# Yotsuei/ClearConverse

Measured on AMD Instinct MI355X. Metric: xRT (audio-sec/wall-sec) end-to-end, 30 s 16 kHz clips, higher is better.
Workload: dtype bf16

## Files before the change

clearconverse_amd/_lib.py:

```python
from __future__ import annotations

import ctypes as C
import os
from pathlib import Path
from typing import Optional

_PKG = Path(__file__).resolve().parent
LIB_PATH = _PKG / "libccx.so"


class CcxError(RuntimeError):
    pass


class WhisperDims(C.Structure):
    _fields_ = [(n, C.c_int) for n in (
        "n_mels", "n_audio_ctx", "n_audio_state", "n_audio_head", "n_audio_layer",
        "n_vocab", "n_text_ctx", "n_text_state", "n_text_head", "n_text_layer")]


class SepformerDims(C.Structure):
    _fields_ = [(n, C.c_int) for n in (
        "n_filters", "kernel", "stride", "d_model", "n_head", "d_ffn", "n_layers", "n_blocks", "segment", "n_spk")]

# ... 59 lines not shown
        + [(n, C.c_int64) for n in ("h_elems", "xin_elems", "y_elems", "qkv_elems", "att_elems", "feats_elems", "fc_elems")]
        + [("rows", C.c_int), ("seq_start", C.POINTER(C.c_int)), ("seq_len", C.POINTER(C.c_int)), ("n_seq", C.c_int),
           ("n_tok", C.c_int), ("d_ffn", C.c_int)]
        + [(n, C.c_void_p) for n in ("ln_g", "ln_b", "gln_g", "gln_b", "wqkv", "bqkv", "wo", "bo", "w1", "b1", "w2", "b2", "wdec")]
        + [(n, C.c_int64) for n in ("ln_elems", "gln_elems", "wqkv_elems", "bqkv_elems", "wo_elems", "bo_elems", "w1_elems",
                                    "b1_elems", "w2_elems", "b2_elems", "wdec_elems")]
        + [("utt_tok0", C.POINTER(C.c_int)), ("utt_L", C.POINTER(C.c_int)), ("utt_T", C.POINTER(C.c_int)), ("n_utt", C.c_int),
           ("segment", C.c_int), ("out", C.c_void_p), ("out_stride", C.c_int64), ("out_elems", C.c_int64)])


SEP_ATTN_BLOCK, SEP_ATTENTION, SEP_FFN, SEP_FINAL_NORM, SEP_DECODER = range(5)


class AlignDesc(C.Structure):
    _fields_ = [
        ("q", C.c_void_p), ("k", C.c_void_p), ("q_elems", C.c_int64), ("k_elems", C.c_int64),
        ("n_seq", C.c_int), ("H", C.c_int), ("Spad", C.c_int),
        ("heads", C.POINTER(C.c_int)), ("n_heads", C.c_int), ("head0", C.c_int), ("t", C.c_int),
        ("Hsel", C.c_int), ("T", C.c_int), ("Mmax", C.c_int),
        ("n_keys", C.POINTER(C.c_int)), ("n_rows", C.POINTER(C.c_int)), ("r0", C.c_int),
        ("P", C.c_void_p), ("A", C.c_void_p), ("P_elems", C.c_int64), ("A_elems", C.c_int64),
        ("text_idx", C.c_void_p), ("time_idx", C.c_void_p), ("path_len", C.c_void_p), ("jump_frame", C.c_void_p),
        ("text_idx_elems", C.c_int64), ("time_idx_elems", C.c_int64), ("path_len_elems", C.c_int64), ("jump_frame_elems", C.c_int64)]


ALIGN_SCORES, ALIGN_MATRIX, ALIGN_DTW = range(3)


_vp, _i, _i64, _f = C.c_void_p, C.c_int, C.c_int64, C.c_float
_ip = C.POINTER(C.c_int)
_i32p = C.POINTER(C.c_int32)
_i64p = C.POINTER(C.c_int64)
_fp = C.POINTER(C.c_float)

PROTOTYPES = {
    "ccx_version": (C.c_char_p, []),
    "ccx_ctx_create": (_i, [_i, C.POINTER(_vp)]),
    "ccx_ctx_destroy": (None, [_vp]),
    "ccx_last_error": (C.c_char_p, [_vp]),
    "ccx_prof_enable": (_i, [_vp, _i]),
    "ccx_prof_count": (_i, [_vp]),
    "ccx_prof_get": (_i, [_vp, _i, C.c_char_p, _i, C.POINTER(C.c_double), C.POINTER(C.c_double), _fp]),
    "ccx_gemm_bf16": (_i, [_vp, _i, _vp, _i64, _vp, _i64, _vp, _vp, _i64, _vp, _i64, _i, _i, _i, _vp]),
    "ccx_gemm_bf16_desc": (_i, [_vp, _i, C.POINTER(GemmDesc), _vp]),
    "ccx_layernorm": (_i, [_vp, _vp, _vp, _vp, _vp, _vp, _i, _i, _f, _vp]),
    "ccx_gather_rows": (_i, [_vp, _vp, _vp, _i, _i, _vp, _i64, _vp]),
    "ccx_peak_normalize": (_i, [_vp, _vp, _vp, _i64, _vp, _i, _f, _vp]),
    "ccx_row_variance": (_i, [_vp, _vp, _i64, _vp, _i, _vp, _vp]),
    "ccx_cross_attention_xa": (_i, [_vp, _vp, _vp, _vp, _vp, _vp, _vp, _i, _i, _i, _i, _i, _vp, _vp]),
    "ccx_cosine_rows": (_i, [_vp, _vp, _vp, _i, _i, _i, _vp, _vp]),
    "ccx_speaker_profiles": (_i, [_vp, _vp, _vp, _vp, _i, _i, _i, _i, _vp, _vp]),
    "ccx_resample_sinc": (_i, [_vp, _vp, _i64, _vp, _i, _i, _i, _i, _vp, _vp, _i64, _vp, _i, _vp]),
    "ccx_enc_attention": (_i, [_vp, _vp, _vp, _vp, _vp, _i, _i, _i, _i, _vp]),
    "ccx_whisper_create": (_i, [_vp, C.POINTER(WhisperDims), _i, C.POINTER(_vp)]),
    "ccx_whisper_destroy": (None, [_vp]),
    "ccx_whisper_set_tensor": (_i, [_vp, C.c_char_p, _vp, _i, _i, _i64p]),
    "ccx_whisper_set_max_audio": (_i, [_vp, C.c_double]),
    "ccx_whisper_share_encoder_scratch": (_i, [_vp, _vp]),
    "ccx_whisper_finalize": (_i, [_vp]),
    "ccx_whisper_set_rules": (_i, [_vp, C.POINTER(DecodeRules)]),
    "ccx_whisper_logmel": (_i, [_vp, _vp, _i64, _ip, _ip, _i, _vp, _vp]),
    "ccx_whisper_set_mel": (_i, [_vp, _vp, _i, _vp]),
    "ccx_whisper_encode": (_i, [_vp, _i, _vp, _vp]),
    "ccx_whisper_decoder_logits": (_i, [_vp, _i32p, _i, _i, _vp, _vp]),
    "ccx_whisper_decode_greedy": (_i, [_vp, _i32p, _i32p, _i, _i, _i, _i32p, _i32p, _fp, _fp, _vp]),
    "ccx_dec_attention_desc": (_i, [_vp, _i, C.POINTER(DecAttnDesc), _vp]),
    "ccx_dec_select_step": (_i, [_vp, C.POINTER(DecSelectDesc), _vp]),
    "ccx_align_op": (_i, [_vp, _i, C.POINTER(AlignDesc), _vp]),
    "ccx_whisper_align": (_i, [_vp, _i32p, _i32p, _i, _i, _i32p, _i32p, _i, _i, _vp, _vp, _i32p, _vp]),
    "ccx_whisper_last_cross_path": (_i, [_vp]),
    "ccx_whisper_prepare_lanes": (_i, [_vp, _vp]),
    "ccx_whisper_trace_lanes": (_i, [_vp, C.c_char_p, _i]),
    "ccx_whisper_decode": (_i, [_vp, _i32p, _i32p, _i, _i, _i, _f, C.c_uint64, _i32p, _i32p, _fp, _fp, _vp]),
    "ccx_sepformer_create": (_i, [_vp, C.POINTER(SepformerDims), _i, _i, C.POINTER(_vp)]),
    "ccx_sepformer_destroy": (None, [_vp]),
    "ccx_sepformer_set_tensor": (_i, [_vp, C.c_char_p, _vp, _i64]),
    "ccx_sepformer_finalize": (_i, [_vp]),
    "ccx_sepformer_separate": (_i, [_vp, _vp, _i64, _ip, _i, _vp, _vp]),
    "ccx_sep_op": (_i, [_vp, _i, C.POINTER(SepDesc), _vp]),
    "ccx_speaker_create": (_i, [_vp, _i, _i, _i, _i, _i64, C.POINTER(_vp)]),
    "ccx_speaker_destroy": (None, [_vp]),
    "ccx_speaker_set_tensor": (_i, [_vp, C.c_char_p, _vp, _i64]),
    "ccx_speaker_finalize": (_i, [_vp]),
    "ccx_speaker_embed": (_i, [_vp, _vp, _i64p, _ip, _i, _vp, _i64p, _ip, _vp, _vp]),
    "ccx_speaker_segment": (_i, [_vp, _vp, _i64p, _ip, _i, _vp, _i64, _ip, _vp]),
    "ccx_resnet_create": (_i, [_vp, _i, _i64, _i, C.POINTER(_vp)]),
    "ccx_resnet_destroy": (None, [_vp]),
    "ccx_resnet_set_tensor": (_i, [_vp, C.c_char_p, _vp, _i64]),
    "ccx_resnet_finalize": (_i, [_vp]),
    "ccx_resnet_embed": (_i, [_vp, _vp, _i64, _i, _i, _vp, _i, _ip, _i, _vp, _vp]),
    "ccx_specgate_create": (_i, [_vp, _i64, _i, _i, C.POINTER(_vp)]),
    "ccx_specgate_destroy": (None, [_vp]),
    "ccx_specgate_reduce": (_i, [_vp, _vp, _i64, _ip, _i, _f, _vp, _vp]),
    "ccx_specgate_reduce_long": (_i, [_vp, _vp, _i64, _f, _vp, _vp]),
    "ccx_specgate_set_clip_noise": (_i, [_vp, _i]),
}

_lib: Optional[C.CDLL] = None


def load() -> C.CDLL:
    global _lib
    if _lib is not None:
        return _lib
    if not LIB_PATH.exists():
        raise CcxError(f"{LIB_PATH} is missing: run `python -m clearconverse_amd.build` "
# ... 71 lines not shown
```

clearconverse_amd/csrc/api.hip:

```cpp
#include <stdarg.h>
#include "../../include/ccx.h"
#include "attention.h"
#include "ccx_common.h"
#include "elementwise.h"
#include "gemm_bf16.h"

static thread_local std::string g_create_error;

int ccx_fail(ccx_ctx* ctx, int code, const char* fmt, ...) {
  char buf[1024];
  va_list ap;
  va_start(ap, fmt);
  vsnprintf(buf, sizeof(buf), fmt, ap);
  va_end(ap);
  if (ctx) {
    std::lock_guard<std::mutex> lk(ctx->mu);
    ctx->last_error = buf;
  } else g_create_error = buf;
  return code;
}

extern "C" {

const char* ccx_version(void) { return "ccx 0.1 (gfx950)"; }
// ... 112 lines not shown
      if (rrow > max_rrow) max_rrow = rrow;
    }
    const long o_need = max_orow < 0 ? 0 : max_orow * p.ldo + Nw;
    CCX_REQUIRE(ctx, o_need <= d->out_elems, "ccx_gemm_bf16_desc: out is written up to element %ld, out_elems=%ld", o_need, (long)d->out_elems);
    const bool res_f32 = epi == EPI_F32_RESID || epi == EPI_F32_GELU_POS || epi == EPI_BF16_LRELU_AFFINE;
    if (res_f32 && p.resid) {
      const long r_need = max_rrow * p.ldr + Nw;
      CCX_REQUIRE(ctx, r_need <= d->resid_elems, "ccx_gemm_bf16_desc: resid is read up to element %ld, resid_elems=%ld", r_need, (long)d->resid_elems);
    }
    if (epi == EPI_BF16_ADD_RELU && p.resid_bf16) {
      const long r_need = max_rrow * p.ldrb + Nw;
      CCX_REQUIRE(ctx, r_need <= d->resid_bf16_elems, "ccx_gemm_bf16_desc: resid_bf16 is read up to element %ld, resid_bf16_elems=%ld", r_need,
                  (long)d->resid_bf16_elems);
    }
  }
  return ccx_launch_gemm(ctx, epi, p, (hipStream_t)stream);
}

int ccx_layernorm(ccx_ctx* ctx, const float* x, const float* gamma, const float* beta, void* out_bf16, float* out_f32,
                  int M, int D, float eps, void* stream) {
  if (!ctx) return CCX_ERR_ARG;
  return ccx_launch_layernorm(ctx, x, D, gamma, beta, (bf16_t*)out_bf16, out_f32, D, M, D, eps, (hipStream_t)stream);
}

int ccx_peak_normalize(ccx_ctx* ctx, const float* x, float* y, int64_t stride, const int* n_samples_dev, int B, float eps, void* stream) {
  if (!ctx) return CCX_ERR_ARG;
  return ccx_launch_peak_normalize(ctx, x, y, (long)stride, n_samples_dev, B, eps, (hipStream_t)stream);
}

int ccx_row_variance(ccx_ctx* ctx, const float* x, int64_t stride, const int* n_samples_dev, int B, float* out, void* stream) {
  if (!ctx) return CCX_ERR_ARG;
  return ccx_launch_row_variance(ctx, x, (long)stride, n_samples_dev, B, out, (hipStream_t)stream);
}

int ccx_cosine_rows(ccx_ctx* ctx, const float* a, const float* b, int R, int D, int b_rows, float* out, void* stream) {
  if (!ctx) return CCX_ERR_ARG;
  return ccx_launch_cosine_rows(ctx, a, b, R, D, b_rows, out, (hipStream_t)stream);
}

int ccx_speaker_profiles(ccx_ctx* ctx, const float* emb, const float* w, const int* spk_dev, int C, int T, int D, int S, float* out, void* stream) {
  if (!ctx) return CCX_ERR_ARG;
  return ccx_launch_speaker_profiles(ctx, emb, w, spk_dev, C, T, D, S, out, (hipStream_t)stream);
}

int ccx_gather_rows(ccx_ctx* ctx, const int64_t* src_ptrs_dev, const int* lens_dev, int n_rows, int max_len, float* dst_dev,
                    int64_t stride, void* stream) {
  if (!ctx) return CCX_ERR_ARG;
  return ccx_launch_gather_rows(ctx, (const long*)src_ptrs_dev, lens_dev, n_rows, max_len, dst_dev, (long)stride, (hipStream_t)stream);
}

int ccx_enc_attention(ccx_ctx* ctx, const void* q, const void* k, const void* vt, void* o, int B, int H, int S, int Spad,
                      void* stream) {
  if (!ctx) return CCX_ERR_ARG;
  return ccx_launch_enc_attention(ctx, (const bf16_t*)q, (const bf16_t*)k, (const bf16_t*)vt, (bf16_t*)o, B, H, S, Spad,
                                  (hipStream_t)stream);
}

}
```

clearconverse_amd/csrc/attention.h:

```cpp
#pragma once
#include "ccx_common.h"

int ccx_launch_enc_attention(ccx_ctx* ctx, const bf16_t* Q, const bf16_t* K, const bf16_t* Vt, bf16_t* O,
                             int B, int n_head, int S, int Spad, hipStream_t stream);
```

clearconverse_amd/csrc/attention.hip:

```cpp
#include <type_traits>
#include "attention.h"

typedef const __attribute__((address_space(1))) void* gptr_t;
typedef __attribute__((address_space(3))) void* lptr_t;

#define ATT_STAGE 16384

__global__ __launch_bounds__(256, 2) void enc_attention_kernel(
    const bf16_t* __restrict__ Q, const bf16_t* __restrict__ Kc, const bf16_t* __restrict__ Vt,
    bf16_t* __restrict__ O, int S, int Spad, int n_head, float scale_log2e, int n_qt) {
  __shared__ __attribute__((aligned(16))) char smem[2 * ATT_STAGE];
  const int tid = threadIdx.x, lane = tid & 63, wave = tid >> 6;
  const int nwg = gridDim.x, orig = blockIdx.x;
  const int xcd = orig & 7, qq = nwg >> 3, rr = nwg & 7;
  const int wg = (xcd < rr ? xcd * (qq + 1) : rr * (qq + 1) + (xcd - rr) * qq) + (orig >> 3);
  const int bh = wg / n_qt;
  const int q0 = (wg - bh * n_qt) * 128 + wave * 32;
  const int l31 = lane & 31, hh = lane >> 5;

  const bf16_t* Qb = Q + (long)bh * Spad * 64;
  const bf16_t* Kb = Kc + (long)bh * Spad * 64;
  const bf16_t* Vb = Vt + (long)bh * 64 * Spad;

  bf16x8 qf[4];
  {
    int qr = q0 + l31; qr = qr < Spad ? qr : Spad - 1;
#pragma unroll
    for (int ds = 0; ds < 4; ds++) qf[ds] = *(const bf16x8*)(Qb + (long)qr * 64 + 16 * ds + 8 * hh);
  }

  const bf16_t* srcK[2];
  const bf16_t* srcV[2];
#pragma unroll
  for (int i = 0; i < 2; i++) {
    const int inst = wave * 2 + i;
    const int r = inst * 8 + (lane >> 3);
    const int c = (lane & 7) ^ ((r >> 1) & 7);
    srcK[i] = Kb + (long)r * 64 + c * 8;
    srcV[i] = Vb + (long)r * Spad + c * 8;
  }
  auto stage = [&](int t, int buf) {
    char* sK = smem + buf * ATT_STAGE;
    char* sV = sK + 8192;
#pragma unroll
    for (int i = 0; i < 2; i++) {
      const int inst = wave * 2 + i;
      __builtin_amdgcn_global_load_lds((gptr_t)(srcK[i] + (long)t * 64 * 64), (lptr_t)(sK + inst * 1024), 16, 0, 0);
      __builtin_amdgcn_global_load_lds((gptr_t)(srcV[i] + (long)t * 64), (lptr_t)(sV + inst * 1024), 16, 0, 0);
    }
  };

  const int prow = (l31 & ~0xC) | (((l31 >> 2) & 1) << 3) | (((l31 >> 3) & 1) << 2);
  int offK[4], offV[4];
#pragma unroll
  for (int s = 0; s < 4; s++) {
    offK[s] = prow * 128 + (((2 * s + hh) ^ ((prow >> 1) & 7)) << 4);
    offV[s] = l31 * 128 + (((2 * s + hh) ^ ((l31 >> 1) & 7)) << 4);
  }

  f32x16 oT[2];
#pragma unroll
  for (int i = 0; i < 16; i++) { oT[0][i] = 0.f; oT[1][i] = 0.f; }
  float m_run = -1e30f, l_run = 0.f;

  const int nT = (S + 63) >> 6;
  const f32x16 zero16 = {0.f, 0.f, 0.f, 0.f, 0.f, 0.f, 0.f, 0.f, 0.f, 0.f, 0.f, 0.f, 0.f, 0.f, 0.f, 0.f};
  auto tile = [&](int t, auto tail_tag) {
    constexpr bool TAIL = decltype(tail_tag)::value;
    const int buf = t & 1;
    if (t + 1 < nT) stage(t + 1, buf ^ 1);
    const char* sK = smem + buf * ATT_STAGE;
    const char* sV = sK + 8192;

    f32x16 sT[2];
#pragma unroll
    for (int kt = 0; kt < 2; kt++) {
#pragma unroll
      for (int ds = 0; ds < 4; ds++) {
        const bf16x8 kf = *(const bf16x8*)(sK + kt * 32 * 128 + offK[ds]);
        sT[kt] = __builtin_amdgcn_mfma_f32_32x32x16_bf16(kf, qf[ds], ds == 0 ? zero16 : sT[kt], 0, 0, 0);
      }
    }
    float mx = -1e30f;
#pragma unroll
    for (int kt = 0; kt < 2; kt++)
#pragma unroll
      for (int r = 0; r < 16; r++) {
        if (TAIL) {
          const int key = t * 64 + kt * 32 + 16 * (r >> 3) + 8 * hh + (r & 7);
          if (key >= S) sT[kt][r] = -INFINITY;
        }
        mx = fmaxf(mx, sT[kt][r]);
      }
    mx = fmaxf(mx, __shfl_xor(mx, 32, 64));
    const float m_new = fmaxf(m_run, mx * scale_log2e);
    const float alpha = __builtin_amdgcn_exp2f(m_run - m_new);
    m_run = m_new;
    float psum = 0.f;
#pragma unroll
    for (int kt = 0; kt < 2; kt++)
#pragma unroll
      for (int r = 0; r < 16; r++) {
        const float pv = __builtin_amdgcn_exp2f(fmaf(sT[kt][r], scale_log2e, -m_new));
        sT[kt][r] = pv;
        psum += pv;
      }
    l_run = l_run * alpha + psum;
    if (__builtin_amdgcn_ballot_w64(alpha != 1.f) != 0) {
#pragma unroll
      for (int i = 0; i < 16; i++) { oT[0][i] *= alpha; oT[1][i] *= alpha; }
    }

    bf16x8 pf[4];
#pragma unroll
    for (int kt = 0; kt < 2; kt++)
#pragma unroll
      for (int s = 0; s < 2; s++) {
        union { bf16x8 v; uint32_t u[4]; } cv;
#pragma unroll
        for (int j = 0; j < 4; j++) cv.u[j] = pack_bf16x2(sT[kt][8 * s + 2 * j], sT[kt][8 * s + 2 * j + 1]);
        pf[2 * kt + s] = cv.v;
      }
#pragma unroll
    for (int dt = 0; dt < 2; dt++)
#pragma unroll
      for (int ks = 0; ks < 4; ks++) {
        const bf16x8 vf = *(const bf16x8*)(sV + dt * 32 * 128 + offV[ks]);
        oT[dt] = __builtin_amdgcn_mfma_f32_32x32x16_bf16(vf, pf[ks], oT[dt], 0, 0, 0);
      }
    __syncthreads();
  };
  stage(0, 0);
  __syncthreads();
  for (int t = 0; t < nT - 1; t++) tile(t, std::false_type{});
  if ((S & 63) != 0) tile(nT - 1, std::true_type{});
  else tile(nT - 1, std::false_type{});

  const float l_tot = l_run + __shfl_xor(l_run, 32, 64);
  const float inv = 1.0f / l_tot;
  const int q = q0 + l31;
  if (q < S) {
    const int b = bh / n_head, h = bh - b * n_head;
    bf16_t* dst = O + ((long)(b * S + q) * n_head + h) * 64;
#pragma unroll
    for (int dt = 0; dt < 2; dt++)
#pragma unroll
      for (int g = 0; g < 4; g++) {
        uint2 v;
        v.x = pack_bf16x2(oT[dt][4 * g + 0] * inv, oT[dt][4 * g + 1] * inv);
        v.y = pack_bf16x2(oT[dt][4 * g + 2] * inv, oT[dt][4 * g + 3] * inv);
        *(uint2*)(dst + dt * 32 + 8 * g + 4 * hh) = v;
      }
  }
}

int ccx_launch_enc_attention(ccx_ctx* ctx, const bf16_t* Q, const bf16_t* K, const bf16_t* Vt, bf16_t* O,
                             int B, int n_head, int S, int Spad, hipStream_t stream) {
  CCX_REQUIRE(ctx, B > 0 && n_head > 0 && S > 0, "enc_attention: empty problem");
  CCX_REQUIRE(ctx, Spad % 64 == 0 && Spad >= S, "enc_attention: Spad=%d must be a multiple of 64 and >= S=%d", Spad, S);
  const float scale_log2e = 0.125f * 1.4426950408889634f;
  const int n_qt = ccx_cdiv(S, 128);
  dim3 grid(n_qt * B * n_head);
  {
    const double bh = (double)B * n_head;
    ccx_prof_scope ps(ctx, stream, "enc_attention_kernel", 4.0 * bh * S * (double)S * 64, 2.0 * bh * S * 64 * 4);
    hipLaunchKernelGGL(enc_attention_kernel, grid, dim3(256), 0, stream, Q, K, Vt, O, S, Spad, n_head, scale_log2e, n_qt);
  }
  CCX_CHECK_LAUNCH(ctx);
  return CCX_OK;
}
```

clearconverse_amd/csrc/whisper.hip:

```cpp
#include <array>
#include <atomic>
#include <map>
#include <chrono>
#include <math.h>
#include "../../include/ccx.h"
#include "align.h"
#include "attention.h"
#include "ccx_common.h"
#include "cross_x.h"
#include "decoder.h"
#include "elementwise.h"
#include "gemm_bf16.h"
#include "logmel.h"
#include "model_store.h"

namespace {

struct EncLayer {
  float *ln1_g, *ln1_b, *ln2_g, *ln2_b;
  bf16_t *Wqkv, *Wo, *W1, *W2;
  float *bqkv, *bo, *b1, *b2;
};
struct DecLayer {
  float *ln1_g, *ln1_b, *lnc_g, *lnc_b, *ln2_g, *ln2_b;
// ... 255 lines not shown

int ccx_whisper_trace_lanes(ccx_whisper* w, const char* path, int level) {
  CCX_REQUIRE(w->ctx, w->finalized, "whisper: trace_lanes before finalize");
  w->stamps_on = path != nullptr && path[0] != 0;
  w->stamp_path = w->stamps_on ? path : "";
  w->stamp_level = level >= 2 ? 2 : 1;
  CCX_HIP(w->ctx, hipMemset(w->stamp_count, 0, ccx_whisper::kMaxLanes * 4));
  for (auto& g : w->graphs) hipGraphExecDestroy(g.second);
  w->graphs.clear();
  return CCX_OK;
}

int ccx_whisper_finalize(ccx_whisper* w) {
  if (!w) return CCX_ERR_ARG;
  CCX_REQUIRE(w->ctx, !w->finalized, "whisper: finalize called twice");
  CCX_HIP(w->ctx, hipSetDevice(w->ctx->device));
  const ccx_whisper_dims& d = w->d;
  const int D = d.n_audio_state, F = 4 * D, B = w->max_batch, S = d.n_audio_ctx, H = d.n_audio_head;
  CCX_TRY(w->store.open_arena((size_t)64 << 20));
  CCX_TRY(build_logmel_tables(w));

  {
    CCX_NEED(w->store, c1w, "encoder.conv1.weight", D, d.n_mels, 3);
    CCX_NEED(w->store, c1b, "encoder.conv1.bias", D);
    CCX_NEED(w->store, c2w, "encoder.conv2.weight", D, D, 3);
    CCX_NEED(w->store, c2b, "encoder.conv2.bias", D);
    CCX_NEED(w->store, pe, "encoder.positional_embedding", S, D);
    CCX_NEED(w->store, lg, "encoder.ln_post.weight", D);
    CCX_NEED(w->store, lb, "encoder.ln_post.bias", D);
    std::vector<float> g1 = conv_to_gemm(*c1w, 256), g2 = conv_to_gemm(*c2w, 3 * D);
    CCX_TRY(w->store.upload_bf16(&w->Wc1, g1));
    CCX_TRY(w->store.upload_bf16(&w->Wc2, g2));
    CCX_TRY(w->store.upload(&w->bc1, c1b->data.data(), D));
    CCX_TRY(w->store.upload(&w->bc2, c2b->data.data(), D));
    CCX_TRY(w->store.upload(&w->enc_pos, pe->data.data(), (size_t)S * D));
    CCX_TRY(w->store.upload(&w->lnp_g, lg->data.data(), D));
    CCX_TRY(w->store.upload(&w->lnp_b, lb->data.data(), D));
  }
  w->enc.resize(d.n_audio_layer);
  const std::vector<float> zerosD(D, 0.f);
  for (int l = 0; l < d.n_audio_layer; l++) {
    const std::string p = "encoder.blocks." + std::to_string(l) + ".";
    EncLayer& L = w->enc[l];
    CCX_NEED(w->store, qw, p + "attn.query.weight", D, D); CCX_NEED(w->store, qbias, p + "attn.query.bias", D);
    CCX_NEED(w->store, kw, p + "attn.key.weight", D, D);
    CCX_NEED(w->store, vw, p + "attn.value.weight", D, D); CCX_NEED(w->store, vbias, p + "attn.value.bias", D);
    CCX_NEED(w->store, ow, p + "attn.out.weight", D, D); CCX_NEED(w->store, obias, p + "attn.out.bias", D);
    CCX_NEED(w->store, l1g, p + "attn_ln.weight", D); CCX_NEED(w->store, l1b, p + "attn_ln.bias", D);
    CCX_NEED(w->store, m0w, p + "mlp.0.weight", F, D); CCX_NEED(w->store, m0b, p + "mlp.0.bias", F);
    CCX_NEED(w->store, m2w, p + "mlp.2.weight", D, F); CCX_NEED(w->store, m2b, p + "mlp.2.bias", D);
    CCX_NEED(w->store, l2g, p + "mlp_ln.weight", D); CCX_NEED(w->store, l2b, p + "mlp_ln.bias", D);
    std::vector<float> wqkv = cat_rows({&qw->data, &kw->data, &vw->data});
    std::vector<float> bqkv = cat_rows({&qbias->data, &zerosD, &vbias->data});
    CCX_TRY(w->store.upload_bf16(&L.Wqkv, wqkv)); CCX_TRY(w->store.upload(&L.bqkv, bqkv));
    CCX_TRY(w->store.upload_bf16(&L.Wo, ow->data)); CCX_TRY(w->store.upload(&L.bo, obias->data.data(), D));
    CCX_TRY(w->store.upload_bf16(&L.W1, m0w->data)); CCX_TRY(w->store.upload(&L.b1, m0b->data.data(), F));
    CCX_TRY(w->store.upload_bf16(&L.W2, m2w->data)); CCX_TRY(w->store.upload(&L.b2, m2b->data.data(), D));
    CCX_TRY(w->store.upload(&L.ln1_g, l1g->data.data(), D)); CCX_TRY(w->store.upload(&L.ln1_b, l1b->data.data(), D));
    CCX_TRY(w->store.upload(&L.ln2_g, l2g->data.data(), D)); CCX_TRY(w->store.upload(&L.ln2_b, l2b->data.data(), D));
  }

  {
    CCX_NEED(w->store, te, "decoder.token_embedding.weight", d.n_vocab, D);
    CCX_NEED(w->store, pe, "decoder.positional_embedding", d.n_text_ctx, D);
    CCX_NEED(w->store, lg, "decoder.ln.weight", D);
    CCX_NEED(w->store, lb, "decoder.ln.bias", D);
    CCX_TRY(w->store.upload(&w->tok_emb_f32, te->data));
    CCX_TRY(w->store.upload_bf16(&w->tok_emb_rm, te->data.data(), (size_t)d.n_vocab * D));
    CCX_TRY(w->store.upload(&w->dec_pos, pe->data));
    CCX_TRY(w->store.upload(&w->lnd_g, lg->data.data(), D));
    CCX_TRY(w->store.upload(&w->lnd_b, lb->data.data(), D));
  }
  w->dec.resize(d.n_text_layer);
  const int Tc = d.n_text_ctx;
  {
    const char* e = getenv("CCX_CROSS_X");
    w->xs_on = (!e || atoi(e) != 0) && d.n_text_state == D && d.n_text_head == H && ccx_xs_supported(D, H);
    w->kv_cap = w->xs_on ? (B < ccx_whisper::kKvSeqs ? B : ccx_whisper::kKvSeqs) : B;
  }
  for (int l = 0; l < d.n_text_layer; l++) {
    const std::string p = "decoder.blocks." + std::to_string(l) + ".";
    DecLayer& L = w->dec[l];
    CCX_NEED(w->store, qw, p + "attn.query.weight", D, D); CCX_NEED(w->store, qbias, p + "attn.query.bias", D);
    CCX_NEED(w->store, kw, p + "attn.key.weight", D, D);
    CCX_NEED(w->store, vw, p + "attn.value.weight", D, D); CCX_NEED(w->store, vbias, p + "attn.value.bias", D);
    CCX_NEED(w->store, ow, p + "attn.out.weight", D, D); CCX_NEED(w->store, obias, p + "attn.out.bias", D);
    CCX_NEED(w->store, l1g, p + "attn_ln.weight", D); CCX_NEED(w->store, l1b, p + "attn_ln.bias", D);
    CCX_NEED(w->store, cqw, p + "cross_attn.query.weight", D, D); CCX_NEED(w->store, cqb, p + "cross_attn.query.bias", D);
    CCX_NEED(w->store, ckw, p + "cross_attn.key.weight", D, D);
    CCX_NEED(w->store, cvw, p + "cross_attn.value.weight", D, D); CCX_NEED(w->store, cvb, p + "cross_attn.value.bias", D);
    CCX_NEED(w->store, cow, p + "cross_attn.out.weight", D, D); CCX_NEED(w->store, cob, p + "cross_attn.out.bias", D);
    CCX_NEED(w->store, lcg, p + "cross_attn_ln.weight", D); CCX_NEED(w->store, lcb, p + "cross_attn_ln.bias", D);
    CCX_NEED(w->store, m0w, p + "mlp.0.weight", F, D); CCX_NEED(w->store, m0b, p + "mlp.0.bias", F);
    CCX_NEED(w->store, m2w, p + "mlp.2.weight", D, F); CCX_NEED(w->store, m2b, p + "mlp.2.bias", D);
    CCX_NEED(w->store, l2g, p + "mlp_ln.weight", D); CCX_NEED(w->store, l2b, p + "mlp_ln.bias", D);
    std::vector<float> wqkv = cat_rows({&qw->data, &kw->data, &vw->data});
    std::vector<float> bqkv = cat_rows({&qbias->data, &zerosD, &vbias->data});
    std::vector<float> wckv = cat_rows({&ckw->data, &cvw->data});
    std::vector<float> bckv = cat_rows({&zerosD, &cvb->data});
    CCX_TRY(up_bf16_packed(w, &L.Wqkv, wqkv.data(), 3 * D, D, 16)); CCX_TRY(w->store.upload(&L.bqkv, bqkv));
    CCX_TRY(up_bf16_packed(w, &L.Wo, ow->data.data(), D, D, 16)); CCX_TRY(w->store.upload(&L.bo, obias->data.data(), D));
    { double sb = 0.0; for (int k = 0; k < D; k++) sb += obias->data[k]; L.bo_mean = (float)(sb / D); }
    CCX_TRY(up_bf16_packed(w, &L.Wcq, cqw->data.data(), D, D, 16)); CCX_TRY(w->store.upload(&L.bcq, cqb->data.data(), D));
    CCX_TRY(w->store.upload_bf16(&L.Wckv, wckv)); CCX_TRY(w->store.upload(&L.bckv, bckv));
    CCX_TRY(up_bf16_packed(w, &L.Wco, cow->data.data(), D, D, 16)); CCX_TRY(w->store.upload(&L.bco, cob->data.data(), D));
    CCX_TRY(up_bf16_packed(w, &L.W1, m0w->data.data(), F, D, 16)); CCX_TRY(w->store.upload(&L.b1, m0b->data.data(), F));
// ... 195 lines not shown
  CCX_REQUIRE(w->ctx, n <= w->kv_cap, "whisper: cross K/V caches hold %d sequences, %d asked for", w->kv_cap, n);
  GemmParams p;
  for (int l = 0; l < d.n_text_layer; l++) {
    const DecLayer& L = w->dec[l];
    memset(&p, 0, sizeof(p));
    p.A = w->xa; p.lda = D; p.W = L.Wckv; p.ldw = D; p.M = n * S; p.N = 2 * D; p.K = D; p.bias = L.bckv;
    p.hk = L.crossK; p.hv = L.crossV; p.d_model = D; p.n_head = H; p.S = S; p.Spad = w->Spad; p.v_transposed = 0;
    p.first_block = 1;
    CCX_TRY(ccx_launch_gemm(w->ctx, EPI_HEADS, p, stream));
  }
  w->kv_ready = n;
  return CCX_OK;
}
static void read_chain_switches(ccx_whisper* w) {
  { const char* e = getenv("CCX_FUSE_CROSS_Q"); w->fuse_cross_q = e ? (atoi(e) != 0) : 1; }
  { const char* e = getenv("CCX_DEC_LNFREE"); w->lnfree = !(e && strcmp(e, "0") == 0); }
  { const char* e = getenv("CCX_XS_FUSE_Q"); w->xs_fuse_q = !e || atoi(e) != 0; }
}
static int select_cross_path(ccx_whisper* w, int B, hipStream_t stream) {
  const char* e = getenv("CCX_CROSS_X_MIN_ROWS");
  const int min_rows = e ? atoi(e) : ccx_whisper::kKvSeqs + 1;
  w->xs_active = w->xs_on && (B >= min_rows || B > w->kv_cap);
  if (w->xs_on && !w->xs_active && w->kv_ready < B) CCX_TRY(project_cross_kv(w, B, stream));
  return CCX_OK;
}

int ccx_whisper_encode(ccx_whisper* w, int B, float* xa_out, void* stream_) {
  if (!w) return CCX_ERR_ARG;
  hipStream_t stream = (hipStream_t)stream_;
  ccx_ctx* ctx = w->ctx;
  CCX_REQUIRE(ctx, w->finalized, "whisper: not finalized");
  CCX_REQUIRE(ctx, B >= 1 && B <= w->max_batch, "whisper_encode: B=%d out of range (max %d)", B, w->max_batch);
  const ccx_whisper_dims& d = w->d;
  const int D = d.n_audio_state, F = 4 * D, S = d.n_audio_ctx, H = d.n_audio_head;
  GemmParams p;
  memset(&p, 0, sizeof(p));
  p.A = w->im2col; p.lda = 256; p.W = w->Wc1; p.ldw = 256; p.M = B * 3000; p.N = D; p.K = 256;
  p.bias = w->bc1; p.out = w->h1; p.ldo = D; p.rpb_in = 3000; p.rpb_out = 3002; p.roff = 1; p.rpb_valid = 3000;
  CCX_TRY(ccx_launch_gemm(ctx, EPI_BF16_GELU, p, stream));
  memset(&p, 0, sizeof(p));
  p.A = w->h1; p.lda = 2 * D; p.W = w->Wc2; p.ldw = 3 * D; p.M = B * 1501; p.N = D; p.K = 3 * D;
  p.bias = w->bc2; p.out = w->x; p.ldo = D; p.resid = w->enc_pos; p.ldr = D; p.resid_mod = S;
  p.rpb_in = 1501; p.rpb_out = S; p.roff = 0; p.rpb_valid = S;
  CCX_TRY(ccx_launch_gemm(ctx, EPI_F32_GELU_POS, p, stream));

  const int M = B * S;
  for (int l = 0; l < d.n_audio_layer; l++) {
    const EncLayer& L = w->enc[l];
    CCX_TRY(ccx_launch_layernorm(ctx, w->x, D, L.ln1_g, L.ln1_b, w->xn, nullptr, D, M, D, 1e-5f, stream));
    memset(&p, 0, sizeof(p));
    p.A = w->xn; p.lda = D; p.W = L.Wqkv; p.ldw = D; p.M = M; p.N = 3 * D; p.K = D; p.bias = L.bqkv;
    p.hq = w->qb; p.hk = w->kb; p.hv = w->vtb; p.d_model = D; p.n_head = H; p.S = S; p.Spad = w->Spad; p.v_transposed = 1;
    CCX_TRY(ccx_launch_gemm(ctx, EPI_HEADS, p, stream));
    CCX_TRY(ccx_launch_enc_attention(ctx, w->qb, w->kb, w->vtb, w->attn, B, H, S, w->Spad, stream));
    memset(&p, 0, sizeof(p));
    p.A = w->attn; p.lda = D; p.W = L.Wo; p.ldw = D; p.M = M; p.N = D; p.K = D; p.bias = L.bo;
    p.out = w->x; p.ldo = D; p.resid = w->x; p.ldr = D;
    CCX_TRY(ccx_launch_gemm(ctx, EPI_F32_RESID, p, stream));
    CCX_TRY(ccx_launch_layernorm(ctx, w->x, D, L.ln2_g, L.ln2_b, w->xn, nullptr, D, M, D, 1e-5f, stream));
    memset(&p, 0, sizeof(p));
    p.A = w->xn; p.lda = D; p.W = L.W1; p.ldw = D; p.M = M; p.N = F; p.K = D; p.bias = L.b1; p.out = w->ffn; p.ldo = F;
    CCX_TRY(ccx_launch_gemm(ctx, EPI_BF16_GELU, p, stream));
    memset(&p, 0, sizeof(p));
    p.A = w->ffn; p.lda = F; p.W = L.W2; p.ldw = F; p.M = M; p.N = D; p.K = F; p.bias = L.b2;
    p.out = w->x; p.ldo = D; p.resid = w->x; p.ldr = D;
    CCX_TRY(ccx_launch_gemm(ctx, EPI_F32_RESID, p, stream));
  }
  CCX_TRY(ccx_launch_layernorm(ctx, w->x, D, w->lnp_g, w->lnp_b, w->xa, xa_out, D, M, D, 1e-5f, stream));
  CCX_TRY(scratch_release(w, stream));
  w->kv_ready = 0;
  if (!w->xs_on) CCX_TRY(project_cross_kv(w, B, stream));
  return CCX_OK;
}

}

namespace {

__global__ void dec_stamp_kernel(unsigned long long* trace, int* count, int cap, int tag) {
  const int i = atomicAdd(count, 1);
  if (i < cap) trace[i] = (__builtin_amdgcn_s_memrealtime() << 8) | (unsigned long long)(tag & 255);
}

__global__ void lane_probe_spin(int* sink, long cycles) {
  const long t0 = __builtin_amdgcn_s_memtime();
  while (__builtin_amdgcn_s_memtime() - t0 < cycles) {}
  if (sink && threadIdx.x == 0) atomicAdd(sink, 1);
}

double lane_probe_time(ccx_whisper* w, hipStream_t a, hipStream_t b) {
  hipStreamSynchronize(a);
  if (b) hipStreamSynchronize(b);
  const auto t0 = std::chrono::steady_clock::now();
  for (int k = 0; k < 4; k++) {
    hipLaunchKernelGGL(lane_probe_spin, dim3(1), dim3(64), 0, a, w->probe_sink, 120000L);
    if (b) hipLaunchKernelGGL(lane_probe_spin, dim3(1), dim3(64), 0, b, w->probe_sink + 1, 120000L);
  }
  hipStreamSynchronize(a);
  if (b) hipStreamSynchronize(b);
  return std::chrono::duration<double, std::micro>(std::chrono::steady_clock::now() - t0).count();
}

const std::vector<hipStream_t>& lane_streams_for(ccx_whisper* w, hipStream_t s0, int want) {
  auto it = w->lane_sets.find(s0);
  if (it != w->lane_sets.end()) return it->second;
  (void)want;
  std::vector<hipStream_t>& set = w->lane_sets[s0];
// ... 617 lines not shown
```

include/ccx.h:

```cpp
#ifndef CCX_H
#define CCX_H
#include <stdint.h>
#ifdef __cplusplus
extern "C" {
#endif

#define CCX_DTYPE_F32 0
#define CCX_DTYPE_BF16 1
#define CCX_DTYPE_F16 2

typedef struct ccx_ctx ccx_ctx;
typedef struct ccx_whisper ccx_whisper;

const char* ccx_version(void);
int ccx_ctx_create(int device, ccx_ctx** out);
void ccx_ctx_destroy(ccx_ctx* ctx);
const char* ccx_last_error(const ccx_ctx* ctx);

int ccx_prof_enable(ccx_ctx* ctx, int on);
int ccx_prof_count(ccx_ctx* ctx);
int ccx_prof_get(ccx_ctx* ctx, int i, char* name_out, int name_cap, double* flops, double* bytes, float* ms);


int ccx_gemm_bf16(ccx_ctx* ctx, int epi, const void* A_dev, int64_t lda, const void* W_dev, int64_t ldw,
                  const float* bias_dev, void* out_dev, int64_t ldo, const float* resid_dev, int64_t ldr,
                  int M, int N, int K, void* stream);

typedef struct ccx_gemm_desc {
  const void* A; const void* W;
  int64_t lda, ldw;
  int M, N, K;
  int ntaps; int64_t a_tap_stride;
  const void* bias;
  const void* out;
  int64_t ldo;
  const void* resid;
  int64_t ldr;
  int resid_mod;
  const void* scale; const void* shift;
  float slope;
  int rpb_in, rpb_out, roff, rpb_valid;
  int img_rows_in, img_rows_valid, img_rows_out;
  const void* resid_bf16; int64_t ldrb;
  const void* hq; const void* hk; const void* hv;
  int d_model, n_head;
  int S, Spad;
  int v_transposed;
  int first_block;
  int64_t a_elems, w_elems, out_elems, resid_elems, resid_bf16_elems, heads_elems;
} ccx_gemm_desc;

int ccx_gemm_bf16_desc(ccx_ctx* ctx, int epi, const ccx_gemm_desc* desc, void* stream);

int ccx_layernorm(ccx_ctx* ctx, const float* x_dev, const float* gamma_dev, const float* beta_dev,
                  void* out_bf16_dev, float* out_f32_dev, int M, int D, float eps, void* stream);

int ccx_gather_rows(ccx_ctx* ctx, const int64_t* src_ptrs_dev, const int* lens_dev, int n_rows, int max_len, float* dst_dev,
                    int64_t stride, void* stream);
int ccx_peak_normalize(ccx_ctx* ctx, const float* x_dev, float* y_dev, int64_t stride, const int* n_samples_dev, int B,
                       float eps, void* stream);
int ccx_cross_attention_xa(ccx_ctx* ctx, const float* q_dev, const float* wk_host, const float* wv_host, const float* bv_host,
                           const uint16_t* xa_dev, const int* row_seq_host, int rows_per_seq, int rows, int n_seq, int n_head, int n_ctx,
                           float* out_dev, void* stream);
int ccx_row_variance(ccx_ctx* ctx, const float* x_dev, int64_t stride, const int* n_samples_dev, int B, float* out_dev, void* stream);
int ccx_cosine_rows(ccx_ctx* ctx, const float* a_dev, const float* b_dev, int R, int D, int b_rows, float* out_dev, void* stream);
int ccx_speaker_profiles(ccx_ctx* ctx, const float* emb_dev, const float* w_dev, const int* spk_dev, int C, int T, int D, int S,
                         float* out_dev, void* stream);

int ccx_resample_sinc(ccx_ctx* ctx, const float* x_dev, int64_t stride_in, const int* n_in_dev, int B, int orig, int new_,
                      int width, const float* kernT_dev, float* y_dev, int64_t stride_out, const int* n_out_dev, int max_out,
                      void* stream);

int ccx_enc_attention(ccx_ctx* ctx, const void* q_dev, const void* k_dev, const void* vt_dev, void* o_dev,
                      int B, int H, int S, int Spad, void* stream);


typedef struct {
  int n_mels, n_audio_ctx, n_audio_state, n_audio_head, n_audio_layer;
  int n_vocab, n_text_ctx, n_text_state, n_text_head, n_text_layer;
} ccx_whisper_dims;

typedef struct {
  int eot, sot, sot_prev, no_speech, no_timestamps, timestamp_begin, blank;
  int max_initial_timestamp_index;
  int n_suppress;
  const int* suppress;
} ccx_decode_rules;

int ccx_whisper_create(ccx_ctx* ctx, const ccx_whisper_dims* dims, int max_batch, ccx_whisper** out);
void ccx_whisper_destroy(ccx_whisper* w);
int ccx_whisper_set_tensor(ccx_whisper* w, const char* name, const void* data, int dtype, int ndim,
                           const int64_t* shape);
int ccx_whisper_set_max_audio(ccx_whisper* w, double seconds);
int ccx_whisper_share_encoder_scratch(ccx_whisper* w, ccx_whisper* donor);
int ccx_whisper_finalize(ccx_whisper* w);
int ccx_whisper_set_rules(ccx_whisper* w, const ccx_decode_rules* rules);

int ccx_whisper_logmel(ccx_whisper* w, const float* audio_dev, int64_t stride, const int* n_samples,
                       const int* seek_frames, int B, float* mel_out_dev, void* stream);
int ccx_whisper_set_mel(ccx_whisper* w, const float* mel_dev, int B, void* stream);
int ccx_whisper_encode(ccx_whisper* w, int B, float* xa_out_dev, void* stream);

int ccx_whisper_decoder_logits(ccx_whisper* w, const int32_t* tokens, int B, int T, float* logits_dev,
                               void* stream);

int ccx_whisper_decode_greedy(ccx_whisper* w, const int32_t* prompt_ids, const int32_t* prompt_lens,
                              int max_prompt, int B, int sample_len, int32_t* tokens_out,
                              int32_t* n_tokens_out, float* sum_logprob_out, float* no_speech_prob_out,
                              void* stream);

int ccx_whisper_decode(ccx_whisper* w, const int32_t* prompt_ids, const int32_t* prompt_lens, int max_prompt, int B,
                       int sample_len, float temperature, uint64_t seed, int32_t* tokens_out, int32_t* n_tokens_out,
                       float* sum_logprob_out, float* no_speech_prob_out, void* stream);

#define CCX_DEC_ATTN_SELF 0
#define CCX_DEC_ATTN_SPLIT 1
#define CCX_DEC_ATTN_STREAM 2
#define CCX_DEC_ATTN_PREFILL 3
#define CCX_DEC_ATTN_FUSED_Q 4
#define CCX_DEC_ATTN_TWO_LAUNCH_Q 5

typedef struct ccx_dec_attn_desc {
  const void* q; const void* k; const void* v;
  int rows, n_seq, H, kv_T;
  int T;
  const int* pos;
  const int* row_seq;
  int rows_per_seq;
// ... 133 lines not shown
```

Baseline: 1670.

## Fold softmax scale into Q weights and use fixed-max encoder attention

Multiplies the encoder Q projection weights and bias by the softmax scale times log2(e) at load time, so attention scores arrive already in the exp2 domain. The encoder attention kernel gains a prescaled path that takes the first tile's row max as a fixed offset, pre-loads it into the MFMA accumulator, and skips the per-tile running max and rescale. If any row's sum overflows, the block falls back to the online-softmax pass. The change also generalises the K/V staging over the wave count, skips the second half of the last tile when it is past S, and raises the occupancy hint to 3. The risks are bf16 rounding of the scaled Q weights and a full second pass whenever the overflow check fires.

```diff
diff --git a/clearconverse_amd/_lib.py b/clearconverse_amd/_lib.py
--- a/clearconverse_amd/_lib.py
+++ b/clearconverse_amd/_lib.py
@@ -135,6 +135,7 @@
     "ccx_speaker_profiles": (_i, [_vp, _vp, _vp, _vp, _i, _i, _i, _i, _vp, _vp]),
     "ccx_resample_sinc": (_i, [_vp, _vp, _i64, _vp, _i, _i, _i, _i, _vp, _vp, _i64, _vp, _i, _vp]),
     "ccx_enc_attention": (_i, [_vp, _vp, _vp, _vp, _vp, _i, _i, _i, _i, _vp]),
+    "ccx_enc_attention_prescaled": (_i, [_vp, _vp, _vp, _vp, _vp, _i, _i, _i, _i, _vp]),
     "ccx_whisper_create": (_i, [_vp, C.POINTER(WhisperDims), _i, C.POINTER(_vp)]),
     "ccx_whisper_destroy": (None, [_vp]),
     "ccx_whisper_set_tensor": (_i, [_vp, C.c_char_p, _vp, _i, _i, _i64p]),
diff --git a/clearconverse_amd/csrc/api.hip b/clearconverse_amd/csrc/api.hip
--- a/clearconverse_amd/csrc/api.hip
+++ b/clearconverse_amd/csrc/api.hip
@@ -188,8 +188,15 @@
 int ccx_enc_attention(ccx_ctx* ctx, const void* q, const void* k, const void* vt, void* o, int B, int H, int S, int Spad,
                       void* stream) {
   if (!ctx) return CCX_ERR_ARG;
-  return ccx_launch_enc_attention(ctx, (const bf16_t*)q, (const bf16_t*)k, (const bf16_t*)vt, (bf16_t*)o, B, H, S, Spad,
+  return ccx_launch_enc_attention(ctx, (const bf16_t*)q, (const bf16_t*)k, (const bf16_t*)vt, (bf16_t*)o, B, H, S, Spad, false,
                                   (hipStream_t)stream);
 }
 
-}
+int ccx_enc_attention_prescaled(ccx_ctx* ctx, const void* q, const void* k, const void* vt, void* o, int B, int H, int S,
+                                int Spad, void* stream) {
+  if (!ctx) return CCX_ERR_ARG;
+  return ccx_launch_enc_attention(ctx, (const bf16_t*)q, (const bf16_t*)k, (const bf16_t*)vt, (bf16_t*)o, B, H, S, Spad, true,
+                                  (hipStream_t)stream);
+}
+
+}
diff --git a/clearconverse_amd/csrc/attention.h b/clearconverse_amd/csrc/attention.h
--- a/clearconverse_amd/csrc/attention.h
+++ b/clearconverse_amd/csrc/attention.h
@@ -1,5 +1,7 @@
 #pragma once
 #include "ccx_common.h"
 
+#define CCX_ENC_ATT_QSCALE (0.125f * 1.4426950408889634f)
+
 int ccx_launch_enc_attention(ccx_ctx* ctx, const bf16_t* Q, const bf16_t* K, const bf16_t* Vt, bf16_t* O,
-                             int B, int n_head, int S, int Spad, hipStream_t stream);
+                             int B, int n_head, int S, int Spad, bool q_prescaled, hipStream_t stream);
diff --git a/clearconverse_amd/csrc/attention.hip b/clearconverse_amd/csrc/attention.hip
--- a/clearconverse_amd/csrc/attention.hip
+++ b/clearconverse_amd/csrc/attention.hip
@@ -6,17 +6,18 @@
 
 #define ATT_STAGE 16384
 
-__global__ __launch_bounds__(256, 2) void enc_attention_kernel(
+template <bool PRE, int NW>
+__device__ __forceinline__ void enc_attention_body(
     const bf16_t* __restrict__ Q, const bf16_t* __restrict__ Kc, const bf16_t* __restrict__ Vt,
-    bf16_t* __restrict__ O, int S, int Spad, int n_head, float scale_log2e, int n_qt) {
-  __shared__ __attribute__((aligned(16))) char smem[2 * ATT_STAGE];
-  const int tid = threadIdx.x, lane = tid & 63, wave = tid >> 6;
+    bf16_t* __restrict__ O, int S, int Spad, int n_head, float scale_log2e, int n_qt, char* smem) {
+  const int tid = threadIdx.x, lane = tid & 63, wave = __builtin_amdgcn_readfirstlane(tid >> 6);
   const int nwg = gridDim.x, orig = blockIdx.x;
   const int xcd = orig & 7, qq = nwg >> 3, rr = nwg & 7;
   const int wg = (xcd < rr ? xcd * (qq + 1) : rr * (qq + 1) + (xcd - rr) * qq) + (orig >> 3);
   const int bh = wg / n_qt;
-  const int q0 = (wg - bh * n_qt) * 128 + wave * 32;
+  const int q0 = (wg - bh * n_qt) * (32 * NW) + wave * 32;
   const int l31 = lane & 31, hh = lane >> 5;
+  const bool has_rows = q0 < S;
 
   const bf16_t* Qb = Q + (long)bh * Spad * 64;
   const bf16_t* Kb = Kc + (long)bh * Spad * 64;
@@ -29,24 +30,31 @@
     for (int ds = 0; ds < 4; ds++) qf[ds] = *(const bf16x8*)(Qb + (long)qr * 64 + 16 * ds + 8 * hh);
   }
 
-  const bf16_t* srcK[2];
-  const bf16_t* srcV[2];
-#pragma unroll
-  for (int i = 0; i < 2; i++) {
-    const int inst = wave * 2 + i;
-    const int r = inst * 8 + (lane >> 3);
+  static_assert(NW % 2 == 0 && NW >= 4 && NW <= 8, "enc_attention: 4, 6 or 8 waves");
+  constexpr int NI = (16 + NW - 1) / NW;
+  const char* gsrc[NI];
+  long tstep[NI];
+  unsigned loff[NI];
+  {
+    const int r = (wave & 1) * 8 + (lane >> 3);
     const int c = (lane & 7) ^ ((r >> 1) & 7);
-    srcK[i] = Kb + (long)r * 64 + c * 8;
-    srcV[i] = Vb + (long)r * Spad + c * 8;
+    const unsigned laneK = ((lane >> 3) * 64 + c * 8) * 2, laneV = ((lane >> 3) * Spad + c * 8) * 2;
+#pragma unroll
+    for (int i = 0; i < NI; i++) {
+      const int j = wave + NW * i;
+      const bool isV = j >= 8;
+      gsrc[i] = isV ? (const char*)(Vb + (long)(j - 8) * 8 * Spad) : (const char*)(Kb + (long)j * 8 * 64);
+      tstep[i] = isV ? 64 * 2 : 64 * 64 * 2;
+      loff[i] = isV ? laneV : laneK;
+    }
   }
   auto stage = [&](int t, int buf) {
-    char* sK = smem + buf * ATT_STAGE;
-    char* sV = sK + 8192;
-#pragma unroll
-    for (int i = 0; i < 2; i++) {
-      const int inst = wave * 2 + i;
-      __builtin_amdgcn_global_load_lds((gptr_t)(srcK[i] + (long)t * 64 * 64), (lptr_t)(sK + inst * 1024), 16, 0, 0);
-      __builtin_amdgcn_global_load_lds((gptr_t)(srcV[i] + (long)t * 64), (lptr_t)(sV + inst * 1024), 16, 0, 0);
+    char* sKV = smem + buf * ATT_STAGE;
+#pragma unroll
+    for (int i = 0; i < NI; i++) {
+      const int j = wave + NW * i;
+      if (j < 16)
+        __builtin_amdgcn_global_load_lds((gptr_t)(gsrc[i] + t * tstep[i] + loff[i]), (lptr_t)(sKV + j * 1024), 16, 0, 0);
     }
   };
 
@@ -65,76 +73,174 @@
 
   const int nT = (S + 63) >> 6;
   const f32x16 zero16 = {0.f, 0.f, 0.f, 0.f, 0.f, 0.f, 0.f, 0.f, 0.f, 0.f, 0.f, 0.f, 0.f, 0.f, 0.f, 0.f};
-  auto tile = [&](int t, auto tail_tag) {
+  auto pv_half = [&](const char* sV, const f32x16& p, int kt) {
+    bf16x8 pf[2];
+#pragma unroll
+    for (int s = 0; s < 2; s++) {
+      union { bf16x8 v; uint32_t u[4]; } cv;
+#pragma unroll
+      for (int j = 0; j < 4; j++) cv.u[j] = pack_bf16x2(p[8 * s + 2 * j], p[8 * s + 2 * j + 1]);
+      pf[s] = cv.v;
+    }
+#pragma unroll
+    for (int s = 0; s < 2; s++)
+#pragma unroll
+      for (int dt = 0; dt < 2; dt++) {
+        const bf16x8 vf = *(const bf16x8*)(sV + dt * 32 * 128 + offV[2 * kt + s]);
+        oT[dt] = __builtin_amdgcn_mfma_f32_32x32x16_bf16(vf, pf[s], oT[dt], 0, 0, 0);
+      }
+  };
+  auto tile = [&](int t, bool on, auto tail_tag) {
     constexpr bool TAIL = decltype(tail_tag)::value;
     const int buf = t & 1;
-    if (t + 1 < nT) stage(t + 1, buf ^ 1);
     const char* sK = smem + buf * ATT_STAGE;
     const char* sV = sK + 8192;
-
-    f32x16 sT[2];
-#pragma unroll
-    for (int kt = 0; kt < 2; kt++) {
-#pragma unroll
-      for (int ds = 0; ds < 4; ds++) {
-        const bf16x8 kf = *(const bf16x8*)(sK + kt * 32 * 128 + offK[ds]);
-        sT[kt] = __builtin_amdgcn_mfma_f32_32x32x16_bf16(kf, qf[ds], ds == 0 ? zero16 : sT[kt], 0, 0, 0);
-      }
-    }
-    float mx = -1e30f;
-#pragma unroll
-    for (int kt = 0; kt < 2; kt++)
-#pragma unroll
-      for (int r = 0; r < 16; r++) {
+    if (!on) {
+      if (t + 1 < nT) stage(t + 1, buf ^ 1);
+    } else {
+      if (t + 1 < nT) stage(t + 1, buf ^ 1);
+      f32x16 sT[2];
+#pragma unroll
+      for (int kt = 0; kt < 2; kt++) {
+#pragma unroll
+        for (int ds = 0; ds < 4; ds++) {
+          const bf16x8 kf = *(const bf16x8*)(sK + kt * 32 * 128 + offK[ds]);
+          sT[kt] = __builtin_amdgcn_mfma_f32_32x32x16_bf16(kf, qf[ds], ds == 0 ? zero16 : sT[kt], 0, 0, 0);
+        }
+      }
+      float mx = -1e30f;
+#pragma unroll
+      for (int kt = 0; kt < 2; kt++)
+#pragma unroll
+        for (int r = 0; r < 16; r++) {
+          if (TAIL) {
+            const int key = t * 64 + kt * 32 + 16 * (r >> 3) + 8 * hh + (r & 7);
+            if (key >= S) sT[kt][r] = -INFINITY;
+          }
+          mx = fmaxf(mx, sT[kt][r]);
+        }
+      mx = fmaxf(mx, __shfl_xor(mx, 32, 64));
+      const float m_new = fmaxf(m_run, PRE ? mx : mx * scale_log2e);
+      const float alpha = __builtin_amdgcn_exp2f(m_run - m_new);
+      m_run = m_new;
+      float psum = 0.f;
+#pragma unroll
+      for (int kt = 0; kt < 2; kt++)
+#pragma unroll
+        for (int r = 0; r < 16; r++) {
+          const float pv = __builtin_amdgcn_exp2f(PRE ? sT[kt][r] - m_new : fmaf(sT[kt][r], scale_log2e, -m_new));
+          sT[kt][r] = pv;
+          psum += pv;
+        }
+      l_run = l_run * alpha + psum;
+      if (__builtin_amdgcn_ballot_w64(alpha != 1.f) != 0) {
+#pragma unroll
+        for (int i = 0; i < 16; i++) { oT[0][i] *= alpha; oT[1][i] *= alpha; }
+      }
+      pv_half(sV, sT[0], 0);
+      pv_half(sV, sT[1], 1);
+    }
+    __syncthreads();
+  };
+  auto run_online = [&](bool on) {
+    stage(0, 0);
+    __syncthreads();
+    for (int t = 0; t < nT - 1; t++) tile(t, on, std::false_type{});
+    if ((S & 63) != 0) tile(nT - 1, on, std::true_type{});
+    else tile(nT - 1, on, std::false_type{});
+  };
+
+  if (PRE) {
+    f32x16 negm = zero16;
+    auto tile_fixed = [&](int t, auto first_tag, auto tail_tag) {
+      constexpr bool FIRST = decltype(first_tag)::value;
+      constexpr bool TAIL = decltype(tail_tag)::value;
+      const int buf = t & 1;
+      const char* sK = smem + buf * ATT_STAGE;
+      const char* sV = sK + 8192;
+      if (!has_rows) {
+        if (t + 1 < nT) stage(t + 1, buf ^ 1);
+      } else {
+        if (t + 1 < nT) stage(t + 1, buf ^ 1);
+        f32x16 sT[2];
+        const bool half1 = !TAIL || t * 64 + 32 < S;
+#pragma unroll
+        for (int kt = 0; kt < 2; kt++) {
+          if (kt == 1 && !half1) {
+#pragma unroll
+            for (int r = 0; r < 16; r++) sT[1][r] = -INFINITY;
+            continue;
+          }
+#pragma unroll
+          for (int ds = 0; ds < 4; ds++) {
+            const bf16x8 kf = *(const bf16x8*)(sK + kt * 32 * 128 + offK[ds]);
+            sT[kt] = __builtin_amdgcn_mfma_f32_32x32x16_bf16(kf, qf[ds], ds == 0 ? (FIRST ? zero16 : negm) : sT[kt], 0, 0, 0);
+          }
+        }
         if (TAIL) {
-          const int key = t * 64 + kt * 32 + 16 * (r >> 3) + 8 * hh + (r & 7);
-          if (key >= S) sT[kt][r] = -INFINITY;
-        }
-        mx = fmaxf(mx, sT[kt][r]);
-      }
-    mx = fmaxf(mx, __shfl_xor(mx, 32, 64));
-    const float m_new = fmaxf(m_run, mx * scale_log2e);
-    const float alpha = __builtin_amdgcn_exp2f(m_run - m_new);
-    m_run = m_new;
-    float psum = 0.f;
-#pragma unroll
-    for (int kt = 0; kt < 2; kt++)
-#pragma unroll
-      for (int r = 0; r < 16; r++) {
-        const float pv = __builtin_amdgcn_exp2f(fmaf(sT[kt][r], scale_log2e, -m_new));
-        sT[kt][r] = pv;
-        psum += pv;
-      }
-    l_run = l_run * alpha + psum;
-    if (__builtin_amdgcn_ballot_w64(alpha != 1.f) != 0) {
-#pragma unroll
-      for (int i = 0; i < 16; i++) { oT[0][i] *= alpha; oT[1][i] *= alpha; }
-    }
-
-    bf16x8 pf[4];
-#pragma unroll
-    for (int kt = 0; kt < 2; kt++)
-#pragma unroll
-      for (int s = 0; s < 2; s++) {
-        union { bf16x8 v; uint32_t u[4]; } cv;
-#pragma unroll
-        for (int j = 0; j < 4; j++) cv.u[j] = pack_bf16x2(sT[kt][8 * s + 2 * j], sT[kt][8 * s + 2 * j + 1]);
-        pf[2 * kt + s] = cv.v;
-      }
-#pragma unroll
-    for (int dt = 0; dt < 2; dt++)
-#pragma unroll
-      for (int ks = 0; ks < 4; ks++) {
-        const bf16x8 vf = *(const bf16x8*)(sV + dt * 32 * 128 + offV[ks]);
-        oT[dt] = __builtin_amdgcn_mfma_f32_32x32x16_bf16(vf, pf[ks], oT[dt], 0, 0, 0);
-      }
-    __syncthreads();
-  };
-  stage(0, 0);
-  __syncthreads();
-  for (int t = 0; t < nT - 1; t++) tile(t, std::false_type{});
-  if ((S & 63) != 0) tile(nT - 1, std::true_type{});
-  else tile(nT - 1, std::false_type{});
+#pragma unroll
+          for (int kt = 0; kt < 2; kt++)
+#pragma unroll
+            for (int r = 0; r < 16; r++) {
+              const int key = t * 64 + kt * 32 + 16 * (r >> 3) + 8 * hh + (r & 7);
+              if (key >= S) sT[kt][r] = -INFINITY;
+            }
+        }
+        if (FIRST) {
+          float mx = sT[0][0];
+#pragma unroll
+          for (int kt = 0; kt < 2; kt++)
+#pragma unroll
+            for (int r = 0; r < 16; r++) mx = fmaxf(mx, sT[kt][r]);
+          mx = fmaxf(mx, __shfl_xor(mx, 32, 64));
+#pragma unroll
+          for (int i = 0; i < 16; i++) { negm[i] = -mx; sT[0][i] -= mx; sT[1][i] -= mx; }
+        }
+#pragma unroll
+        for (int kt = 0; kt < 2; kt++) {
+          if (kt == 1 && !half1) continue;
+#pragma unroll
+          for (int r = 0; r < 16; r++) {
+            const float pv = __builtin_amdgcn_exp2f(sT[kt][r]);
+            sT[kt][r] = pv;
+            l_run += pv;
+          }
+          pv_half(sV, sT[kt], kt);
+        }
+      }
+      __syncthreads();
+    };
+    stage(0, 0);
+    __syncthreads();
+    if (nT == 1) {
+      if ((S & 63) != 0) tile_fixed(0, std::true_type{}, std::true_type{});
+      else tile_fixed(0, std::true_type{}, std::false_type{});
+    } else {
+      tile_fixed(0, std::true_type{}, std::false_type{});
+      for (int t = 1; t < nT - 1; t++) tile_fixed(t, std::false_type{}, std::false_type{});
+      if ((S & 63) != 0) tile_fixed(nT - 1, std::false_type{}, std::true_type{});
+      else tile_fixed(nT - 1, std::false_type{}, std::false_type{});
+    }
+    const float l_chk = l_run + __shfl_xor(l_run, 32, 64);
+    const bool redo = has_rows && __builtin_amdgcn_ballot_w64(q0 + l31 < S && !(l_chk <= 0x1p100f)) != 0;
+    int* vote = (int*)smem;
+    if (lane == 0) vote[wave] = redo;
+    __syncthreads();
+    int any_redo = 0;
+#pragma unroll
+    for (int i = 0; i < NW; i++) any_redo |= vote[i];
+    __syncthreads();
+    if (any_redo) {
+      if (redo) {
+#pragma unroll
+        for (int i = 0; i < 16; i++) { oT[0][i] = 0.f; oT[1][i] = 0.f; }
+        l_run = 0.f;
+      }
+      run_online(redo);
+    }
+  } else {
+    run_online(has_rows);
+  }
 
   const float l_tot = l_run + __shfl_xor(l_run, 32, 64);
   const float inv = 1.0f / l_tot;
@@ -154,17 +260,36 @@
   }
 }
 
+constexpr int kEncAttWaves = 4;
+__global__ __launch_bounds__(64 * kEncAttWaves, 3) void enc_attention_kernel(
+    const bf16_t* __restrict__ Q, const bf16_t* __restrict__ Kc, const bf16_t* __restrict__ Vt,
+    bf16_t* __restrict__ O, int S, int Spad, int n_head, int n_qt) {
+  __shared__ __attribute__((aligned(16))) char smem[2 * ATT_STAGE];
+  enc_attention_body<true, kEncAttWaves>(Q, Kc, Vt, O, S, Spad, n_head, 1.f, n_qt, smem);
+}
+
+__global__ __launch_bounds__(256, 2) void enc_attention_unscaled_kernel(
+    const bf16_t* __restrict__ Q, const bf16_t* __restrict__ Kc, const bf16_t* __restrict__ Vt,
+    bf16_t* __restrict__ O, int S, int Spad, int n_head, float scale_log2e, int n_qt) {
+  __shared__ __attribute__((aligned(16))) char smem[2 * ATT_STAGE];
+  enc_attention_body<false, 4>(Q, Kc, Vt, O, S, Spad, n_head, scale_log2e, n_qt, smem);
+}
+
 int ccx_launch_enc_attention(ccx_ctx* ctx, const bf16_t* Q, const bf16_t* K, const bf16_t* Vt, bf16_t* O,
-                             int B, int n_head, int S, int Spad, hipStream_t stream) {
+                             int B, int n_head, int S, int Spad, bool q_prescaled, hipStream_t stream) {
   CCX_REQUIRE(ctx, B > 0 && n_head > 0 && S > 0, "enc_attention: empty problem");
   CCX_REQUIRE(ctx, Spad % 64 == 0 && Spad >= S, "enc_attention: Spad=%d must be a multiple of 64 and >= S=%d", Spad, S);
-  const float scale_log2e = 0.125f * 1.4426950408889634f;
-  const int n_qt = ccx_cdiv(S, 128);
+  const int nw = q_prescaled ? kEncAttWaves : 4;
+  const int n_qt = ccx_cdiv(S, 32 * nw);
   dim3 grid(n_qt * B * n_head);
   {
     const double bh = (double)B * n_head;
     ccx_prof_scope ps(ctx, stream, "enc_attention_kernel", 4.0 * bh * S * (double)S * 64, 2.0 * bh * S * 64 * 4);
-    hipLaunchKernelGGL(enc_attention_kernel, grid, dim3(256), 0, stream, Q, K, Vt, O, S, Spad, n_head, scale_log2e, n_qt);
+    if (q_prescaled)
+      hipLaunchKernelGGL(enc_attention_kernel, grid, dim3(64 * nw), 0, stream, Q, K, Vt, O, S, Spad, n_head, n_qt);
+    else
+      hipLaunchKernelGGL(enc_attention_unscaled_kernel, grid, dim3(256), 0, stream, Q, K, Vt, O, S, Spad, n_head,
+                         CCX_ENC_ATT_QSCALE, n_qt);
   }
   CCX_CHECK_LAUNCH(ctx);
   return CCX_OK;
diff --git a/clearconverse_amd/csrc/whisper.hip b/clearconverse_amd/csrc/whisper.hip
--- a/clearconverse_amd/csrc/whisper.hip
+++ b/clearconverse_amd/csrc/whisper.hip
@@ -331,6 +331,8 @@
     CCX_NEED(w->store, l2g, p + "mlp_ln.weight", D); CCX_NEED(w->store, l2b, p + "mlp_ln.bias", D);
     std::vector<float> wqkv = cat_rows({&qw->data, &kw->data, &vw->data});
     std::vector<float> bqkv = cat_rows({&qbias->data, &zerosD, &vbias->data});
+    for (size_t i = 0; i < (size_t)D * D; i++) wqkv[i] *= CCX_ENC_ATT_QSCALE;
+    for (int i = 0; i < D; i++) bqkv[i] *= CCX_ENC_ATT_QSCALE;
     CCX_TRY(w->store.upload_bf16(&L.Wqkv, wqkv)); CCX_TRY(w->store.upload(&L.bqkv, bqkv));
     CCX_TRY(w->store.upload_bf16(&L.Wo, ow->data)); CCX_TRY(w->store.upload(&L.bo, obias->data.data(), D));
     CCX_TRY(w->store.upload_bf16(&L.W1, m0w->data)); CCX_TRY(w->store.upload(&L.b1, m0b->data.data(), F));
@@ -632,7 +634,7 @@
     p.A = w->xn; p.lda = D; p.W = L.Wqkv; p.ldw = D; p.M = M; p.N = 3 * D; p.K = D; p.bias = L.bqkv;
     p.hq = w->qb; p.hk = w->kb; p.hv = w->vtb; p.d_model = D; p.n_head = H; p.S = S; p.Spad = w->Spad; p.v_transposed = 1;
     CCX_TRY(ccx_launch_gemm(ctx, EPI_HEADS, p, stream));
-    CCX_TRY(ccx_launch_enc_attention(ctx, w->qb, w->kb, w->vtb, w->attn, B, H, S, w->Spad, stream));
+    CCX_TRY(ccx_launch_enc_attention(ctx, w->qb, w->kb, w->vtb, w->attn, B, H, S, w->Spad, true, stream));
     memset(&p, 0, sizeof(p));
     p.A = w->attn; p.lda = D; p.W = L.Wo; p.ldw = D; p.M = M; p.N = D; p.K = D; p.bias = L.bo;
     p.out = w->x; p.ldo = D; p.resid = w->x; p.ldr = D;
diff --git a/include/ccx.h b/include/ccx.h
--- a/include/ccx.h
+++ b/include/ccx.h
@@ -74,6 +74,9 @@
 int ccx_enc_attention(ccx_ctx* ctx, const void* q_dev, const void* k_dev, const void* vt_dev, void* o_dev,
                       int B, int H, int S, int Spad, void* stream);
 
+int ccx_enc_attention_prescaled(ccx_ctx* ctx, const void* q_dev, const void* k_dev, const void* vt_dev, void* o_dev,
+                                int B, int H, int S, int Spad, void* stream);
+
 
 typedef struct {
   int n_mels, n_audio_ctx, n_audio_state, n_audio_head, n_audio_layer;
```

After: 1684, median of 6. No clear change (+0.8%).
